# NVlabs/intrinsic3d

Measured on NVIDIA H100. Metric: gauss_newton_iterations_per_sec, higher is better.
Workload: dtype f32

## Files before the change

include/i3d_c_api.h:

```cpp
#ifndef I3D_C_API_H_
#define I3D_C_API_H_

#include <stdint.h>
#include "i3d_types.h"

#ifdef __cplusplus
extern "C" {
#endif

typedef struct I3DEngine I3DEngine;

int         i3d_abi_version(void);
uint64_t    i3d_sizeof_params(void);
uint64_t    i3d_sizeof_iter_info(void);

void        i3d_default_params(I3DParams* p);

int         i3d_engine_create(int device, I3DEngine** out);
void        i3d_engine_destroy(I3DEngine* e);
const char* i3d_last_error(const I3DEngine* e);

int         i3d_upload_grid(I3DEngine* e, int64_t n, const int32_t* xyz, const double* sdf0,
                            const double* sdf_refined, const double* albedo, const float* weight,
                            const uint8_t* rgb, float voxel_size);
// ... 47 lines not shown
int         i3d_mode_colors(I3DEngine* e, int32_t sdf_source, int32_t color_mode, uint8_t* rgb);
int         i3d_download_mesh(I3DEngine* e, float* xyz, uint8_t* rgb, int32_t* faces);

#define I3D_KEYFRAME_CHUNK 32
int         i3d_keyframe_scores(I3DEngine* e, int32_t F, int32_t W, int32_t H, const uint8_t* bgr, double* scores);
int         i3d_upload_rgbd_frames(I3DEngine* e, int32_t F, int32_t W, int32_t H, const uint8_t* bgr, const float* depth, const float* lum);
int         i3d_use_rgbd_level(I3DEngine* e, int32_t lvl, int32_t* W_out, int32_t* H_out);

int         i3d_sensor_frames_begin(I3DEngine* e, const I3DFusionCamera* depth_cam, const I3DFusionCamera* color_cam, int32_t capacity);
int         i3d_sensor_frames_add(I3DEngine* e, int32_t F, const float* depth, const uint8_t* bgr);
int32_t     i3d_sensor_num_frames(const I3DEngine* e);
int         i3d_sensor_keyframe_scores(I3DEngine* e, double* scores);
int         i3d_fusion_integrate_sensor(I3DEngine* e, int32_t n, const int32_t* ids, const float* pose_cam_to_world,
                                        const float* pose_world_to_cam);
int         i3d_select_rgbd_frames(I3DEngine* e, int32_t n, const int32_t* ids);

int         i3d_comm_unique_id(uint8_t id128[128]);
int         i3d_comm_init(I3DEngine* e, int32_t rank, int32_t world, const uint8_t id128[128]);
int         i3d_comm_p2p_export(I3DEngine* e, uint8_t handle64[64]);
int         i3d_comm_p2p_connect(I3DEngine* e, const uint8_t* handles );

int         i3d_set_shard(I3DEngine* e, int64_t voxel_begin, int64_t voxel_end);

double      i3d_phase_ms(const I3DEngine* e, const char* name);
int         i3d_debug_set_kernel_timers(I3DEngine* e, int level);
int64_t     i3d_phase_count(const I3DEngine* e, const char* name);
int64_t     i3d_debug_num_slots(const I3DEngine* e);
int         i3d_debug_set_keep_raw_jacobian(I3DEngine* e, int keep);
int         i3d_debug_get_rows(I3DEngine* e, int32_t* voxel, int32_t* frame, double* residual,
                               double* raw_weight, float* jac_colmajor);
int         i3d_debug_get_observations(I3DEngine* e, int32_t K, int32_t* frames, float* weights,
                                       uint8_t* active);
int         i3d_debug_get_step(I3DEngine* e, double* step, uint8_t* free_mask, double* col_scale);
int         i3d_debug_get_normal_equations(I3DEngine* e, float* b, float* s, float* jtj, float* cam_acc);
int         i3d_debug_apply_operator(I3DEngine* e, const float* v, float* q);
int64_t     i3d_debug_fusion_num_voxels(const I3DEngine* e);
int         i3d_debug_get_fusion_volume(I3DEngine* e, int32_t* xyz, float* sdf, float* weight, uint8_t* rgb);
int         i3d_debug_get_frames(I3DEngine* e, float* lum, float* depth, uint8_t* bgr);

#ifdef __cplusplus
}
#endif
#endif
```

intrinsic3d_b200/csrc/i3d_engine.cu:

```cuda
#include <cuda_runtime.h>
#include <dlfcn.h>

#include <algorithm>
#include <chrono>
#include <climits>
#include <cmath>
#include <cstdarg>
#include <cstdio>
#include <cstdlib>
#include <cstring>
#include <map>
#include <string>
#include <vector>

#include "../../include/i3d_c_api.h"
#include "i3d_kernels.cuh"
#include "i3d_lighting.cuh"
#include "i3d_recolor.cuh"
#include "i3d_gridops.cuh"
#include "i3d_fusion.cuh"
#include "i3d_frames.cuh"
#include "i3d_mesh.h"

#include <cub/device/device_radix_sort.cuh>
// ... 100 lines not shown
    Dev<float> Rt;
    Dev<FramePose> pose_ctx, pose_ctx_c;
    Dev<int32_t> obs_frame, row_frame;
    Dev<float> obs_w;
    Dev<float4> Jt;
    Dev<float2> Jtail;
    Dev<double> row_res, row_wraw;
    Dev<float> ea_w;
    Dev<double> lap;
    Dev<float> cam_acc;
    Dev<double> minv, type_w;
    Dev<int> fail_flag;
    Dev<float> v_bg, v_cg, v_s, v_jtj, v_b, v_x, v_r, v_z, v_p, v_ps, v_qg, v_tr, v_delta;
    Dev<double> v_bgd, v_cgd, v_qgd, cam_accd;
    Dev<CgCtl> ctl;
    Dev<double> red_partials, red_out;
    Dev<unsigned int> red_counters;
    size_t max_blocks = 0;
    bool keep_raw = false;
    Dev<float> dbg_v;
    I3DParams last_params{};
    bool have_iter = false;
    std::map<std::string, Phase> phases;
    cudaEvent_t ev[16];
    std::vector<cudaEvent_t> ev_pool;
    struct TimedLaunch { int a, b; const char* name; };
    std::vector<TimedLaunch> timed;
    size_t ev_used = 0;
    int64_t launches = 0;
    int64_t host_syncs = 0;
    int timer_level = 0;
    Dev<IterDev> iter_dev;
    int last_cg_iterations = 4, prev_cg_iterations = 4;
    Dev<uint8_t> color;
    bool have_color = false;
    Dev<unsigned long long> recolor_counts;
    Dev<int32_t> sv_table, sv_index, sv_nbr;
    Dev<int> sv_scalars, sv_deg;
    Dev<double> sv_acc, sv_work;
    Dev<I3DLightingInfo> sv_info;
    Dev<uint8_t> sh_has;
    int sv_S = 0;
    double* sv_x = nullptr;
    SubvolGrid sv_grid{};
    bool fu_active = false;
    I3DFusionParams fu_p{};
    uint64_t fu_cap = 0;
    int64_t fu_n = 0;
    Dev<unsigned long long> fu_keys; Dev<unsigned> fu_vals;
    Dev<int32_t> fu_x, fu_y, fu_z; Dev<float> fu_sdf, fu_w, fu_sdf2, fu_w2; Dev<uchar4> fu_rgb;
    Dev<int> fu_ctl;
    Dev<float> fu_depth_in, fu_depth, fu_nrm; Dev<uint8_t> fu_bgr;
    Dev<unsigned long long> fu_sk, fu_sk2; Dev<int32_t> fu_si, fu_si2; Dev<uint8_t> fu_cub;
    Dev<uint8_t> kf_bgr; Dev<double> kf_partials, kf_scores;
    int st_F = 0, st_W = 0, st_H = 0;
    Dev<float> st_lum, st_depth, st_tmp[4]; Dev<uint8_t> st_bgr;
    int sn_cap = 0, sn_F = 0;
    I3DFusionCamera sn_dcam{}, sn_ccam{};
    Dev<float> sn_depth; Dev<uint8_t> sn_bgr; Dev<int32_t> sn_ids;
    bool have_mesh = false;
    int64_t mesh_V = 0, mesh_F = 0;
    float* mesh_vpos = nullptr; uint8_t* mesh_vcol = nullptr; int3* mesh_faces = nullptr;
    Dev<uint8_t> ms_case, ms_keep, ms_cub; Dev<int32_t> ms_cnt, ms_sel; Dev<int64_t> ms_off; Dev<unsigned long long> ms_cubes, ms_best;
    Dev<float> ms_cpos, ms_vpos, ms_vpos2; Dev<uint8_t> ms_ccol, ms_vcol, ms_vcol2;
    Dev<uint32_t> ms_klo, ms_klo2; Dev<unsigned long long> ms_khi, ms_khi2;
    Dev<int32_t> ms_perm, ms_perm2, ms_first, ms_fid, ms_head, ms_seg, ms_cvid, ms_parent, ms_used, ms_newid;
// ... 419 lines not shown
    pdl_launch(e, k_pack, blocks_for(threads), kThreads, 0, shv, v0, v1, extra_f, n_extra_f, extra_d, n_extra_d, e->xbuf.p, e->ctl.p, respect_done);
    NK(g_nccl.AllReduce(e->xbuf.p, e->xbuf.p, total, NCCL_FLOAT64, NCCL_SUM, e->comm, e->stream));
    pdl_launch(e, k_unpack, blocks_for(threads), kThreads, 0, shv, v0, v1, extra_f, n_extra_f, extra_d, n_extra_d, e->xbuf.p, e->ctl.p, respect_done);
    e->launches += 2;
    if (epilogue_kind >= 0) { pdl_launch(e, k_epilogue, 1, 32, 0, e->ctl.p, extra_d, epilogue_kind, respect_done); e->launches += 1; }
}

size_t apply_smem_bytes(int F, int K)
{
    return static_cast<size_t>((6 * F + 9 + 15) & ~15) * sizeof(double) + static_cast<size_t>(14 + 6 * K) * kThreads * sizeof(float);
}

size_t accum_smem_bytes(int F, int K)
{
    return static_cast<size_t>((CamAccLayout{F}.size() + 15) & ~15) * sizeof(double) + static_cast<size_t>(K) * 8 * kThreads * sizeof(float);
}

int check_frame_limit(I3DEngine* e, int F, int K)
{
    int optin = 0;
    CK(cudaDeviceGetAttribute(&optin, cudaDevAttrMaxSharedMemoryPerBlockOptin, e->device));
    cudaFuncAttributes fa_acc{}, fa_app{};
    CK(cudaFuncGetAttributes(&fa_acc, k_eg_accum));
    CK(cudaFuncGetAttributes(&fa_app, k_eg_apply<APPLY_CG>));
    const size_t lim = static_cast<size_t>(optin);
    auto fits = [&](int f) { return fa_acc.sharedSizeBytes + accum_smem_bytes(f, K) <= lim && fa_app.sharedSizeBytes + apply_smem_bytes(f, K) <= lim; };
    if (fits(F)) return 0;
    int fmax = 0;
    while (fits(fmax + 1)) ++fmax;
    return fail(e, "i3d_gn_iteration: %d frames at K = %d observations need %zu bytes of shared memory per block in k_eg_accum (device limit %d): "
                   "at most %d frames at K = %d", F, K, fa_acc.sharedSizeBytes + accum_smem_bytes(F, K), optin, fmax, K);
}

void launch_operator(I3DEngine* e, const GridView& g, const RegView& rv, const EgRows& rows, const SolveVecs& sv, const Shard& sh, const float* vin,
                     float dmin, float dmax, int is_cg_iteration, bool sample_timing = false)
{
    if (rows.n_active > 0)
    {
        KernelTimer kt(e, "k_eg_apply", 0);
        pdl_launch(e, k_eg_apply<APPLY_CG>, blocks_for(rows.n_active), kThreads, apply_smem_bytes(e->F, rows.K), g, rows, rv, sv, sv.ps, e->ctl.p, 1, e->site(SITE_EG_APPLY));
    }
    e->launches += 2;
    {
        KernelTimer kt(e, "k_op_partial");
        pdl_launch(e, (k_op_partial<APPLY_CG, 4>), blocks_for(static_cast<size_t>((e->held_count() + 3) / 4)), kThreads, 0, 
            g, rv, sv, sh, e->held_count(), vin, sv.ps, e->type_w.p, dmin, dmax, e->ctl.p, 1, e->site(SITE_OP_POST), e->site(SITE_EG_APPLY).out, is_cg_iteration);
    }
    if (e->world > 1)
    {
        KernelTimer kt(e, "exchange");
        exchange(e, sv.qg, nullptr, sv.qg + 2 * e->n, 6 * e->F + 9, e->site(SITE_OP_POST).out, 1, 1, is_cg_iteration ? EPI_OPERATOR_CG : -1);
    }
}

int gn_iteration_impl(I3DEngine* e, const I3DParams& P, I3DIterInfo& info)
{
    std::memset(&info, 0, sizeof(info));
    if (e->n <= 0) return fail(e, "i3d_gn_iteration: no grid uploaded");
    if (e->F <= 0) return fail(e, "i3d_gn_iteration: no frames uploaded");
    if (!e->have_cam) return fail(e, "i3d_gn_iteration: camera not set");
    if (!e->have_sh) return fail(e, "i3d_gn_iteration: SH coefficients not set");
    if (e->world > 1 && !e->shard_ready) return fail(e, "i3d_gn_iteration: world > 1 but i3d_set_shard was not called after the grid/frames upload");
    int K = P.num_observations;
    if (K <= 0 || K > e->F) K = e->F;
    if (K > I3D_MAX_OBS) return fail(e, "i3d_gn_iteration: num_observations (%d) exceeds I3D_MAX_OBS (%d)", K, I3D_MAX_OBS);
    if (P.lm_steps < 1) return fail(e, "i3d_gn_iteration: lm_steps < 1");
    if (P.residual_reset_period < 1) return fail(e, "i3d_gn_iteration: residual_reset_period < 1");
    if (check_frame_limit(e, e->F, K) != 0) return 1;
    e->K = K;
    e->last_params = P;
    e->phases.clear(); e->timed.clear(); e->ev_used = 0; e->launches = 0; e->host_syncs = 0;
    const int64_t n = e->n;
    const int F = e->F;
    const bool multi = e->world > 1;
    cudaStream_t st = e->stream;
    ensure_vectors(e);
    e->iter_dev.ensure(1);
    const Shard sh = e->shard();
    const int64_t own = sh.own_end - sh.own_begin;
    const int64_t hc = e->held_count();
    const size_t U = static_cast<size_t>(e->U());
    Timer t_total(e, "total", 0);
    auto sync = [&]() { CK(cudaStreamSynchronize(st)); e->host_syncs += 1; };

    Timer t_sel(e, "select", 1);
// ... 98 lines not shown
    }
    if (multi) exchange(e, e->v_bg.p, e->v_cg.p, e->cam_acc.p, lay.size(), e->red_out.p, 2 * kSiteVals, 0);
    pdl_launch(e, k_type_weights, 1, 32, 0, e->iter_dev.p, e->site(SITE_BUILD).out, e->site(SITE_REG).out, P, n, e->type_w.p);
    if (S > 0) pdl_launch(e, k_row_weights, blocks_for(S), kThreads, 0, rows, e->type_w.p);
    SolveVecs sv = solve_vecs(e);
    pdl_launch(e, k_finish_problem, blocks_for(static_cast<size_t>((hc + 3) / 4)), kThreads, 0, g, rv, sv, sh, hc, e->type_w.p, e->cam_acc.p, P.fix_poses, P.fix_intrinsics,
                                                                              P.fix_distortion, P.gradient_tolerance, e->site(SITE_FINISH), e->cam);
    allreduce_scalars(e, e->site(SITE_FINISH).out, 3, -1, 0);
    pdl_launch(e, k_iter_finish, 1, 32, 0, e->iter_dev.p, e->site(SITE_FINISH).out, P);
    e->launches += 5;
    t_build.stop();
    e->have_iter = true;
    if (P.build_only)
    {
        IterDev hb{};
        CK(cudaMemcpyAsync(&hb, e->iter_dev.p, sizeof(hb), cudaMemcpyDeviceToHost, st));
        sync();
        CK(cudaGetLastError());
        info = hb.info;
        t_total.stop();
        return 0;
    }

    Timer t_solve(e, "solve", 3);
    const float dmin = static_cast<float>(P.min_lm_diagonal), dmax = static_cast<float>(std::min(P.max_lm_diagonal, 3.0e38));
    const unsigned upd_blocks = blocks_for(static_cast<size_t>((sh.held_voxel_unknowns() + 3) / 4 + F + 2));
    auto launch_update = [&](bool init, int refresh) {
        if (init) pdl_launch(e, (k_cg_update<true, 4>), upd_blocks, kThreads, 0, sv, sh, e->minv.p, dmin, dmax, e->ctl.p, refresh, e->site(SITE_UPDATE));
        else pdl_launch(e, (k_cg_update<false, 4>), upd_blocks, kThreads, 0, sv, sh, e->minv.p, dmin, dmax, e->ctl.p, refresh, e->site(SITE_UPDATE));
        e->launches += 1;
    };
    const unsigned vec_blocks = blocks_for(static_cast<size_t>(hc));
    const int max_it = P.forced_cg_iterations > 0 ? P.forced_cg_iterations : P.max_linear_solver_iterations;
    int enq = 0;
    auto enqueue_pcg = [&](int count) {
        for (int bidx = 0; bidx < count && enq < max_it; ++bidx)
        {
            ++enq;
            const bool refresh = (enq % P.residual_reset_period == 0);
            {
                KernelTimer kt(e, "k_cg_dir");
                pdl_launch(e, k_cg_dir4, blocks_for(static_cast<size_t>((hc + 3) / 4)), kThreads, 0, sv, sh, hc, e->ctl.p);
                e->launches += 1;
            }
            launch_operator(e, g, rv, rows, sv, sh, sv.p, dmin, dmax, 1, enq == 1);
            if (refresh)
            {
                pdl_launch(e, k_x_update, vec_blocks, kThreads, 0, sv, sh, hc, e->ctl.p);
                CK(cudaMemsetAsync(e->v_qg.p, 0, U * sizeof(float), st));
                pdl_launch(e, k_scale_vec, vec_blocks, kThreads, 0, sv, sh, hc, sv.x, 1.0f, sv.ps, e->ctl.p, 1);
                e->launches += 2;
                launch_operator(e, g, rv, rows, sv, sh, sv.x, dmin, dmax, 0);
                launch_update(false, 1);
            }
            else
            {
                KernelTimer kt(e, "k_cg_update");
                launch_update(false, 0);
            }
            if (multi) allreduce_scalars(e, e->site(SITE_UPDATE).out, 3, EPI_UPDATE, 1);
        }
    };
    auto enqueue_decision = [&]() {
        Timer t_cand(e, "candidate", 5);
        CK(cudaMemsetAsync(e->red_out.p + SITE_CAND * kSiteVals, 0, 3 * kSiteVals * sizeof(double), st));
        pdl_launch(e, k_candidate, vec_blocks, kThreads, 0, g, sv, sh, hc, 0, e->cam, e->c_sdf, e->c_alb, e->c_cam, e->v_delta.p, e->ctl.p, e->site(SITE_CAND));
        GridView gc = e->grid_view(e->c_sdf, e->c_alb);
        pdl_launch(e, k_frame_pose, blocks_for(F, 64), 64, 0, F, e->c_cam, e->pose_ctx_c.p);
        CamView cvc{e->c_cam, e->pose_ctx_c.p, F};
        if (n_active > 0)
        {
            KernelTimer kt(e, "k_eg_cost", 0);
            launch_eg_rows<ROWS_COST>(e, gc, cvc, rows, nullptr, nullptr);
        }
        pdl_launch(e, k_reg_cost, blocks_for(static_cast<size_t>(own)), kThreads, 0, gc, rv, sh, e->c_sdf, e->c_alb, e->site(SITE_REG_COST));
        if (multi) allreduce_scalars(e, e->red_out.p + SITE_CAND * kSiteVals, 3 * kSiteVals, -1, 0);
        pdl_launch(e, k_lm_decide, 1, 32, 0, e->iter_dev.p, e->ctl.p, e->fail_flag.p, e->site(SITE_CAND).out, e->site(SITE_EG_COST).out,
                                      e->site(SITE_REG_COST).out, e->type_w.p, P);
        e->launches += 5;
    };
    IterDev h{};
    for (int it = 1; it <= P.lm_steps; ++it)
    {
        Timer t_pcg(e, "pcg", 4);
        pdl_launch(e, k_lm_begin, 1, 32, 0, e->iter_dev.p, e->ctl.p, e->fail_flag.p, P);
        pdl_launch(e, k_cam_precond, blocks_for(static_cast<size_t>(F) + 2, 64), 64, 0, sv, e->cam_acc.p, e->type_w.p, e->ctl.p, dmin, dmax, e->minv.p, e->fail_flag.p);
        e->launches += 2;
        launch_update(true, 0);
        if (multi) allreduce_scalars(e, e->site(SITE_UPDATE).out, 3, EPI_UPDATE_INIT, 0);
        enq = 0;
        enqueue_pcg(P.forced_cg_iterations > 0 ? P.forced_cg_iterations : std::max(e->last_cg_iterations, e->prev_cg_iterations));
        t_pcg.stop();
        while (true)
        {
            enqueue_decision();
            CK(cudaMemcpyAsync(&h, e->iter_dev.p, sizeof(h), cudaMemcpyDeviceToHost, st));
            sync();
            CK(cudaGetLastError());
            if (!h.pcg_unfinished || h.state != LM_RUNNING) break;
            Timer t_more(e, "pcg", 4);
            enqueue_pcg(2);
        }
        if (h.info.lm_iterations >= 1)
        {
            e->prev_cg_iterations = e->last_cg_iterations;
            e->last_cg_iterations = std::max(1, h.info.cg_iterations[std::min(h.info.lm_iterations - 1, I3D_MAX_LM_STEPS - 1)]);
        }
        if (h.state != LM_RUNNING) break;
    }
    info = h.info;
    if (h.precond_fail) e->error = "camera preconditioner block not SPD";
    if (h.state == LM_ACCEPTED)
    {
        if (multi)
        {
            pdl_launch(e, k_mask_owned, blocks_for(U), kThreads, 0, sv, sh, e->v_delta.p);
            NK(g_nccl.AllReduce(e->v_delta.p, e->v_delta.p, U, NCCL_FLOAT32, NCCL_SUM, e->comm, st));
            pdl_launch(e, k_candidate, blocks_for(U), kThreads, 0, g, sv, sh, static_cast<int64_t>(U), 1, e->cam, e->c_sdf, e->c_alb, e->c_cam, e->v_delta.p, e->ctl.p,
                                                           e->site(SITE_CAND));
            sync();
            e->launches += 2;
// ... 227 lines not shown
}

extern "C" {

int i3d_abi_version(void) { return I3D_ABI_VERSION; }
uint64_t i3d_sizeof_params(void) { return sizeof(I3DParams); }
uint64_t i3d_sizeof_iter_info(void) { return sizeof(I3DIterInfo); }

void i3d_default_params(I3DParams* p)
{
    std::memset(p, 0, sizeof(*p));
    p->lambda[0] = 0.2; p->lambda[1] = 80.0; p->lambda[2] = 120.0; p->lambda[3] = 0.1;
    p->use_er = p->use_es = p->use_ea = 1;
    p->occlusion_distance = 0.02f; p->num_observations = 5; p->lm_steps = 50;
    p->initial_trust_region_radius = 1e4; p->max_trust_region_radius = 1e16; p->min_trust_region_radius = 1e-32;
    p->min_relative_decrease = 1e-3; p->min_lm_diagonal = 1e-6; p->max_lm_diagonal = 1e32; p->eta = 0.1;
    p->function_tolerance = 1e-6; p->gradient_tolerance = 1e-10; p->parameter_tolerance = 1e-8;
    p->max_linear_solver_iterations = 500; p->min_linear_solver_iterations = 0; p->residual_reset_period = 10;
    p->max_consecutive_invalid_steps = 5;
}

int i3d_engine_create(int device, I3DEngine** out)
{
    *out = nullptr;
    int count = 0;
    cudaError_t err = cudaGetDeviceCount(&count);
    if (err != cudaSuccess || count <= 0) return fail(nullptr, "i3d_engine_create: no CUDA device available (%s); this engine has no CPU fallback", cudaGetErrorString(err));
    if (device < 0 || device >= count) return fail(nullptr, "i3d_engine_create: device %d out of range (%d devices)", device, count);
    cudaDeviceProp prop;
    if (cudaGetDeviceProperties(&prop, device) != cudaSuccess) return fail(nullptr, "i3d_engine_create: cannot query device %d", device);
    if (prop.major != 9 || prop.minor != 0) return fail(nullptr, "i3d_engine_create: device %d is sm_%d%d; this library is built for sm_90a (H100) only", device, prop.major, prop.minor);
    I3DEngine* e = new I3DEngine();
    e->device = device;
    const int rc = guarded(e, [&]() {
        CK(cudaStreamCreateWithFlags(&e->stream, cudaStreamNonBlocking));
        for (auto& ev : e->ev) CK(cudaEventCreate(&ev));
        e->ev_pool.resize(4096);
        for (auto& ev : e->ev_pool) CK(cudaEventCreate(&ev));
        return 0;
    });
    if (rc != 0) { g_create_error = e->error; delete e; return rc; }
    *out = e;
    return 0;
}

void i3d_engine_destroy(I3DEngine* e)
{
    if (!e) return;
    cudaSetDevice(e->device);
    cudaStreamSynchronize(e->stream);
    for (size_t r = 0; r < e->peer_base.size(); ++r)
        if (static_cast<int>(r) != e->rank && e->peer_base[r]) cudaIpcCloseMemHandle(e->peer_base[r]);
    if (e->comm && g_nccl.CommDestroy) g_nccl.CommDestroy(e->comm);
    for (auto& ev : e->ev) cudaEventDestroy(ev);
    for (auto& ev : e->ev_pool) cudaEventDestroy(ev);
    if (e->ms_ev_ready) for (auto& ev : e->ms_ev) cudaEventDestroy(ev);
    cudaStreamDestroy(e->stream);
    delete e;
}

const char* i3d_last_error(const I3DEngine* e) { return e ? e->error.c_str() : g_create_error.c_str(); }

int i3d_upload_grid(I3DEngine* e, int64_t n, const int32_t* xyz, const double* sdf0, const double* sdf_refined, const double* albedo,
                    const float* weight, const uint8_t* rgb, float voxel_size)
{
    if (!e) return 1;
// ... 1079 lines not shown
        {
            std::vector<std::pair<std::pair<float, int>, int>> ord;
            for (int k = 0; k < K; ++k)
            {
                const size_t s = static_cast<size_t>(k) * e->stride + a;
                if (fr[s] >= 0) ord.push_back({{w[s], fr[s]}, k});
            }
            std::sort(ord.begin(), ord.end(), [](const auto& x, const auto& y) { return x.first > y.first; });
            for (size_t k = 0; k < ord.size(); ++k)
            {
                if (frames) frames[static_cast<size_t>(act[a]) * K + k] = ord[k].first.second;
                if (weights) weights[static_cast<size_t>(act[a]) * K + k] = ord[k].first.first;
            }
        }
        return 0;
    });
}

int i3d_debug_get_step(I3DEngine* e, double* step, uint8_t* free_mask, double* col_scale)
{
    if (!e || !e->have_iter) return fail(e, "i3d_debug_get_step: no iteration yet");
    return guarded(e, [&]() {
        const size_t U = static_cast<size_t>(e->U());
        std::vector<float> d(U), s(U);
        CK(cudaMemcpyAsync(d.data(), e->v_delta.p, U * sizeof(float), cudaMemcpyDeviceToHost, e->stream));
        CK(cudaMemcpyAsync(s.data(), e->v_s.p, U * sizeof(float), cudaMemcpyDeviceToHost, e->stream));
        CK(cudaStreamSynchronize(e->stream));
        for (size_t j = 0; j < U; ++j)
        {
            if (step) step[j] = d[j];
            if (free_mask) free_mask[j] = s[j] != 0.0f;
            if (col_scale) col_scale[j] = s[j];
        }
        return 0;
    });
}

int i3d_debug_get_normal_equations(I3DEngine* e, float* b, float* s, float* jtj, float* cam_acc)
{
    if (!e || !e->have_iter) return fail(e, "i3d_debug_get_normal_equations: no iteration yet");
    return guarded(e, [&]() {
        const size_t U = static_cast<size_t>(e->U());
        cudaStream_t st = e->stream;
        if (b) CK(cudaMemcpyAsync(b, e->v_b.p, U * sizeof(float), cudaMemcpyDeviceToHost, st));
        if (s) CK(cudaMemcpyAsync(s, e->v_s.p, U * sizeof(float), cudaMemcpyDeviceToHost, st));
        if (jtj) CK(cudaMemcpyAsync(jtj, e->v_jtj.p, U * sizeof(float), cudaMemcpyDeviceToHost, st));
        if (cam_acc) CK(cudaMemcpyAsync(cam_acc, e->cam_acc.p, CamAccLayout{e->F}.size() * sizeof(float), cudaMemcpyDeviceToHost, st));
        CK(cudaStreamSynchronize(st));
        return 0;
    });
}

int i3d_debug_apply_operator(I3DEngine* e, const float* v, float* q)
{
    if (!e || !e->have_iter) return fail(e, "i3d_debug_apply_operator: no iteration yet");
    if (!v || !q) return fail(e, "i3d_debug_apply_operator: NULL vector");
    if (e->world > 1) return fail(e, "i3d_debug_apply_operator: single GPU only");
    return guarded(e, [&]() {
        cudaStream_t st = e->stream;
        const size_t U = static_cast<size_t>(e->U());
        const I3DParams& P = e->last_params;
        e->dbg_v.ensure(U);
        CgCtl saved{}, running{};
        CK(cudaMemcpyAsync(&saved, e->ctl.p, sizeof(CgCtl), cudaMemcpyDeviceToHost, st));
        CK(cudaStreamSynchronize(st));
        running = saved; running.done = 0; running.inv_radius = 0.0;
// ... 56 lines not shown
```

intrinsic3d_b200/csrc/i3d_kernels.cuh:

```cuda
#pragma once
#include <cuda_runtime.h>
#include <stdint.h>
#include <limits.h>
#include "i3d_math.cuh"
#include "i3d_grid.cuh"
#include "../../include/i3d_types.h"

namespace i3d
{

enum : uint8_t { FL_VALID = 1, FL_ACTIVE = 2, FL_RING = 4, FL_FREE_SDF = 8, FL_FREE_ALB = 16, FL_ES_JAC = 32, FL_ROW = 64  };

struct Shard
{
    int64_t own_begin, own_end;
    int64_t hv0, hv1;
    int cam_owner;
    int defer;
    int64_t loc_begin, loc_end;
    __device__ __forceinline__ bool owns_voxel(int64_t v) const { return v >= own_begin && v < own_end; }
    __device__ __forceinline__ bool owns_unknown(int64_t j, int64_t n) const
    {
        return j < n ? owns_voxel(j) : (j < 2 * n ? owns_voxel(j - n) : cam_owner != 0);
    }
    __host__ __device__ __forceinline__ int64_t held_voxel_unknowns() const { return 2 * (hv1 - hv0); }
    __device__ __forceinline__ int64_t unknown(int64_t t, int64_t n) const
    {
        const int64_t L = hv1 - hv0;
        return t < L ? hv0 + t : (t < 2 * L ? n + hv0 + (t - L) : 2 * n + (t - 2 * L));
    }
    __device__ __forceinline__ bool vec4(int64_t e0, int64_t n, int64_t* j0) const
    {
        const int64_t L = hv1 - hv0;
        if (e0 + 4 > 2 * L) return false;
// ... 1759 lines not shown
            a0 += static_cast<double>(rr[i]) * ssum;
        }
        if (sh.cam_owner) { acc[0] = a0; acc[1] = a1; acc[2] = a2; }
    }
    if (grid_reduce<3>(acc, site) && threadIdx.x == 0 && !sh.defer) epilogue_update(ctl, site.out[0], site.out[1], site.out[2], INIT);
}

__global__ void __launch_bounds__(kThreads)
k_cg_dir4(SolveVecs sv, Shard sh, int64_t count, const CgCtl* __restrict__ ctl)
{
    pdl_prologue();
    if (ctl->done) return;
    const int64_t e0 = (blockIdx.x * static_cast<int64_t>(blockDim.x) + threadIdx.x) * 4;
    if (e0 >= count) return;
    const float beta = static_cast<float>(ctl->beta);
    int64_t j0 = 0;
    if (sh.vec4(e0, sv.n, &j0))
    {
        float z[4], p[4], s4[4], ps[4];
        ld4(sv.z, j0, z); ld4(sv.p, j0, p); ld4(sv.s, j0, s4);
#pragma unroll
        for (int i = 0; i < 4; ++i) { p[i] = (beta == 0.0f) ? z[i] : z[i] + beta * p[i]; ps[i] = s4[i] * p[i]; }
        st4(sv.p, j0, p); st4(sv.ps, j0, ps);
    }
    else
        for (int64_t t = e0; t < e0 + 4 && t < count; ++t)
        {
            const int64_t j = sh.unknown(t, sv.n);
            const float p = (beta == 0.0f) ? sv.z[j] : sv.z[j] + beta * sv.p[j];
            sv.p[j] = p; sv.ps[j] = sv.s[j] * p;
        }
}

struct ShareView
{
    int64_t n_shared;
    const int32_t* slist;
    const uint8_t* held;
};

__global__ void k_pack(ShareView sh, const float* __restrict__ v0, const float* __restrict__ v1, const float* __restrict__ extra_f, int n_extra_f,
                       const double* __restrict__ extra_d, int n_extra_d, double* __restrict__ xbuf, const CgCtl* __restrict__ ctl, int respect_done)
{
    pdl_prologue();
    if (respect_done && ctl->done) return;
    const int64_t t = blockIdx.x * static_cast<int64_t>(blockDim.x) + threadIdx.x;
    const int64_t nv = v1 ? 2 : 1;
    if (t < sh.n_shared)
    {
        const int32_t j = sh.slist[t];
        const bool h = sh.held[j] != 0;
        xbuf[t] = h ? static_cast<double>(v0[j]) : 0.0;
        if (v1) xbuf[sh.n_shared + t] = h ? static_cast<double>(v1[j]) : 0.0;
    }
    else if (t < sh.n_shared + n_extra_f) xbuf[nv * sh.n_shared + (t - sh.n_shared)] = static_cast<double>(extra_f[t - sh.n_shared]);
    else if (t < sh.n_shared + n_extra_f + n_extra_d) xbuf[nv * sh.n_shared + (t - sh.n_shared)] = extra_d[t - sh.n_shared - n_extra_f];
}

__global__ void k_unpack(ShareView sh, float* __restrict__ v0, float* __restrict__ v1, float* __restrict__ extra_f, int n_extra_f,
                         double* __restrict__ extra_d, int n_extra_d, const double* __restrict__ xbuf, const CgCtl* __restrict__ ctl, int respect_done)
{
    pdl_prologue();
    if (respect_done && ctl->done) return;
    const int64_t t = blockIdx.x * static_cast<int64_t>(blockDim.x) + threadIdx.x;
    const int64_t nv = v1 ? 2 : 1;
    if (t < sh.n_shared)
// ... 348 lines not shown
```

intrinsic3d_b200/engine.py:

```python
from __future__ import annotations

import ctypes as C
import os

import numpy as np

from .ctypes_defs import (I3DFusionCamera, I3DFusionParams, I3DIterInfo, I3DLightingInfo, I3DLightingParams, I3DMeshInfo, I3DMeshParams,
                          I3DParams)

_HERE = os.path.dirname(os.path.abspath(__file__))
LIB_PATH = os.environ.get("I3D_LIB", os.path.join(_HERE, "libi3d_b200.so"))
_LIB = None

EXPORTED_SYMBOLS = [
    "i3d_abi_version", "i3d_sizeof_params", "i3d_sizeof_iter_info", "i3d_default_params",
    "i3d_engine_create", "i3d_engine_destroy", "i3d_last_error",
    "i3d_upload_grid", "i3d_upload_voxel_params", "i3d_upload_frames", "i3d_set_camera", "i3d_set_sh",
    "i3d_gn_iteration", "i3d_download_state",
    "i3d_sizeof_lighting_params", "i3d_sizeof_lighting_info", "i3d_default_lighting_params", "i3d_estimate_lighting",
    "i3d_lighting_num_subvolumes", "i3d_download_lighting", "i3d_download_voxel_sh",
    "i3d_upload_color_frames", "i3d_recompute_colors", "i3d_download_colors",
    "i3d_num_voxels", "i3d_clear_voxels_outside_thin_shell", "i3d_upsample_grid", "i3d_download_grid",
    "i3d_sizeof_fusion_params", "i3d_default_fusion_params", "i3d_fusion_begin", "i3d_fusion_integrate", "i3d_fusion_finish",
    "i3d_keyframe_scores", "i3d_upload_rgbd_frames", "i3d_use_rgbd_level",
    "i3d_sensor_frames_begin", "i3d_sensor_frames_add", "i3d_sensor_num_frames", "i3d_sensor_keyframe_scores", "i3d_fusion_integrate_sensor",
    "i3d_select_rgbd_frames",
    "i3d_sizeof_mesh_info", "i3d_extract_mesh", "i3d_download_mesh", "i3d_extract_mesh_colored", "i3d_mode_colors",
    "i3d_comm_unique_id", "i3d_comm_init", "i3d_comm_p2p_export", "i3d_comm_p2p_connect", "i3d_set_shard",
    "i3d_phase_ms", "i3d_phase_count", "i3d_debug_set_kernel_timers", "i3d_debug_num_slots", "i3d_debug_set_keep_raw_jacobian",
    "i3d_debug_get_rows", "i3d_debug_get_observations", "i3d_debug_get_step", "i3d_debug_get_normal_equations",
    "i3d_debug_apply_operator", "i3d_debug_fusion_num_voxels", "i3d_debug_get_fusion_volume", "i3d_debug_get_frames",
]
KEYFRAME_CHUNK = 32
COLOR_MODES = {"": 0, "normals": 1, "lap": 2, "lum": 3, "lum_grad": 4, "albedo": 5, "shading_sv": 6, "shading_sv_const": 7, "chroma": 8}


def load_library():
    global _LIB
    if _LIB is not None:
        return _LIB
    if not os.path.exists(LIB_PATH):
        raise RuntimeError(f"{LIB_PATH} not found: build it with intrinsic3d_b200/csrc/build.sh "
                           "(__graft_entry__.build()); there is no CPU fallback")
    L = C.CDLL(LIB_PATH)
    L.i3d_abi_version.restype = C.c_int
    L.i3d_sizeof_params.restype = C.c_uint64
    L.i3d_sizeof_iter_info.restype = C.c_uint64
    L.i3d_last_error.restype = C.c_char_p
    L.i3d_last_error.argtypes = [C.c_void_p]
    L.i3d_phase_ms.restype = C.c_double
    L.i3d_phase_ms.argtypes = [C.c_void_p, C.c_char_p]
    L.i3d_phase_count.restype = C.c_int64
    L.i3d_phase_count.argtypes = [C.c_void_p, C.c_char_p]
    L.i3d_debug_num_slots.restype = C.c_int64
    L.i3d_debug_num_slots.argtypes = [C.c_void_p]
    L.i3d_sizeof_lighting_params.restype = C.c_uint64
    L.i3d_sizeof_lighting_info.restype = C.c_uint64
    L.i3d_lighting_num_subvolumes.restype = C.c_int64
    L.i3d_lighting_num_subvolumes.argtypes = [C.c_void_p]
    L.i3d_num_voxels.restype = C.c_int64
    L.i3d_num_voxels.argtypes = [C.c_void_p]
    L.i3d_sizeof_fusion_params.restype = C.c_uint64
    L.i3d_debug_fusion_num_voxels.restype = C.c_int64
# ... 326 lines not shown

    def phase_count(self, name: str) -> int:
        return int(self.L.i3d_phase_count(self.h, name.encode()))

    def set_kernel_timers(self, level: int):
        self.L.i3d_debug_set_kernel_timers(self.h, C.c_int(int(level)))

    def debug_rows(self, want_jac=True):
        S = int(self.L.i3d_debug_num_slots(self.h))
        voxel = np.empty(S, np.int32)
        frame = np.empty(S, np.int32)
        res = np.empty(S, np.float64)
        w = np.empty(S, np.float64)
        J = np.empty((29, S), np.float32) if want_jac else None
        self._check(self.L.i3d_debug_get_rows(self.h, _p(voxel, C.c_int32), _p(frame, C.c_int32), _p(res, C.c_double), _p(w, C.c_double),
                                              _p(J, C.c_float)))
        return dict(voxel=voxel, frame=frame, residual=res, raw_weight=w, J=J)

    def debug_observations(self, K: int):
        fr = np.empty((self.n, K), np.int32)
        w = np.empty((self.n, K), np.float32)
        act = np.empty(self.n, np.uint8)
        self._check(self.L.i3d_debug_get_observations(self.h, C.c_int32(K), _p(fr, C.c_int32), _p(w, C.c_float), _p(act, C.c_uint8)))
        return fr, w, act

    def debug_step(self):
        U = 2 * self.n + 6 * self.F + 9
        st = np.zeros(U, np.float64)
        fm = np.zeros(U, np.uint8)
        cs = np.zeros(U, np.float64)
        self._check(self.L.i3d_debug_get_step(self.h, _p(st, C.c_double), _p(fm, C.c_uint8), _p(cs, C.c_double)))
        return st, fm, cs

    def debug_normal_equations(self):
        U = 2 * self.n + 6 * self.F + 9
        b, s, jtj = np.empty(U, np.float32), np.empty(U, np.float32), np.empty(U, np.float32)
        cam = np.empty(33 * self.F + 43, np.float32)
        self._check(self.L.i3d_debug_get_normal_equations(self.h, _p(b, C.c_float), _p(s, C.c_float), _p(jtj, C.c_float), _p(cam, C.c_float)))
        return dict(b=b, s=s, jtj=jtj, cam_acc=cam)

    def debug_apply_operator(self, v):
        U = 2 * self.n + 6 * self.F + 9
        v = np.ascontiguousarray(v, np.float32)
        assert v.shape == (U,)
        q = np.empty(U, np.float32)
        self._check(self.L.i3d_debug_apply_operator(self.h, _p(v, C.c_float), _p(q, C.c_float)))
        return q


def shard_range(n: int, rank: int, world: int, align: int = 512):
    if world <= 1:
        return 0, n
    per = -(-n // world)
    per = -(-per // align) * align
    b = min(n, rank * per)
    e = min(n, (rank + 1) * per)
    if rank == world - 1:
        e = n
    return b, e


def cut_ranges(cost, world: int, align: int = 64):
    import torch
    n = int(cost.shape[0])
    c = torch.cumsum(cost.to(torch.float64), 0)
    total = float(c[-1].item()) if n > 0 else 0.0
# ... 105 lines not shown
```

Before: 133.9.

## Fuse PCG operator epilogue, update and direction into one cooperative kernel

```diff
diff --git a/include/i3d_c_api.h b/include/i3d_c_api.h
--- a/include/i3d_c_api.h
+++ b/include/i3d_c_api.h
@@ -103,6 +103,7 @@
 int         i3d_debug_get_observations(I3DEngine* e, int32_t K, int32_t* frames, float* weights,
                                        uint8_t* active);
 int         i3d_debug_get_step(I3DEngine* e, double* step, uint8_t* free_mask, double* col_scale);
+int         i3d_debug_get_pcg_vectors(I3DEngine* e, float* x, float* p);
 int         i3d_debug_get_normal_equations(I3DEngine* e, float* b, float* s, float* jtj, float* cam_acc);
 int         i3d_debug_apply_operator(I3DEngine* e, const float* v, float* q);
 int64_t     i3d_debug_fusion_num_voxels(const I3DEngine* e);
diff --git a/intrinsic3d_b200/csrc/i3d_engine.cu b/intrinsic3d_b200/csrc/i3d_engine.cu
--- a/intrinsic3d_b200/csrc/i3d_engine.cu
+++ b/intrinsic3d_b200/csrc/i3d_engine.cu
@@ -156,6 +156,9 @@
     int timer_level = 0;
     Dev<IterDev> iter_dev;
     int last_cg_iterations = 4, prev_cg_iterations = 4;
+    bool pcg_fused = true;
+    int64_t step_n = -1;
+    unsigned step_grid = 0; int step_K = 0; size_t step_smem = 0;
     Dev<uint8_t> color;
     bool have_color = false;
     Dev<unsigned long long> recolor_counts;
@@ -641,15 +644,21 @@
                    "at most %d frames at K = %d", F, K, fa_acc.sharedSizeBytes + accum_smem_bytes(F, K), optin, fmax, K);
 }
 
+void launch_eg_apply(I3DEngine* e, const GridView& g, const RegView& rv, const EgRows& rows, const SolveVecs& sv)
+{
+    if (rows.n_active > 0)
+    {
+        KernelTimer kt(e, "k_eg_apply", 0);
+        pdl_launch(e, k_eg_apply<APPLY_CG>, blocks_for(rows.n_active), kThreads, apply_smem_bytes(e->F, rows.K), g, rows, rv, sv, sv.ps, e->ctl.p, 1, e->site(SITE_EG_APPLY));
+    }
+    e->launches += 1;
+}
+
 void launch_operator(I3DEngine* e, const GridView& g, const RegView& rv, const EgRows& rows, const SolveVecs& sv, const Shard& sh, const float* vin,
                      float dmin, float dmax, int is_cg_iteration, bool sample_timing = false)
 {
-    if (rows.n_active > 0)
-    {
-        KernelTimer kt(e, "k_eg_apply", 0);
-        pdl_launch(e, k_eg_apply<APPLY_CG>, blocks_for(rows.n_active), kThreads, apply_smem_bytes(e->F, rows.K), g, rows, rv, sv, sv.ps, e->ctl.p, 1, e->site(SITE_EG_APPLY));
-    }
-    e->launches += 2;
+    launch_eg_apply(e, g, rv, rows, sv);
+    e->launches += 1;
     {
         KernelTimer kt(e, "k_op_partial");
         pdl_launch(e, (k_op_partial<APPLY_CG, 4>), blocks_for(static_cast<size_t>((e->held_count() + 3) / 4)), kThreads, 0, 
@@ -660,6 +669,55 @@
         KernelTimer kt(e, "exchange");
         exchange(e, sv.qg, nullptr, sv.qg + 2 * e->n, 6 * e->F + 9, e->site(SITE_OP_POST).out, 1, 1, is_cg_iteration ? EPI_OPERATOR_CG : -1);
     }
+}
+
+bool plan_cg_step(I3DEngine* e)
+{
+    if (e->step_n == e->n) return e->step_grid > 0;
+    e->step_n = e->n; e->step_grid = 0;
+    int sms = 0, optin = 0;
+    CK(cudaDeviceGetAttribute(&sms, cudaDevAttrMultiProcessorCount, e->device));
+    CK(cudaDeviceGetAttribute(&optin, cudaDevAttrMaxSharedMemoryPerBlockOptin, e->device));
+    cudaFuncAttributes fa0{}, fa1{};
+    CK(cudaFuncGetAttributes(&fa0, k_cg_step<false>));
+    CK(cudaFuncGetAttributes(&fa1, k_cg_step<true>));
+    const size_t dyn_max = static_cast<size_t>(optin) - std::max(fa0.sharedSizeBytes, fa1.sharedSizeBytes);
+    CK(cudaFuncSetAttribute(k_cg_step<false>, cudaFuncAttributeMaxDynamicSharedMemorySize, static_cast<int>(dyn_max)));
+    CK(cudaFuncSetAttribute(k_cg_step<true>, cudaFuncAttributeMaxDynamicSharedMemorySize, static_cast<int>(dyn_max)));
+    const int64_t items = (e->n + 3) / 4;
+    for (int bps = 2048 / kStepThreads; bps >= 1; --bps)
+    {
+        const int64_t threads = static_cast<int64_t>(bps) * sms * kStepThreads;
+        const int64_t K = (items + threads - 1) / threads;
+        const size_t smem = static_cast<size_t>(K) * kStepSlots * kStepThreads * sizeof(float);
+        if (smem > dyn_max) break;
+        int occ0 = 0, occ1 = 0;
+        CK(cudaOccupancyMaxActiveBlocksPerMultiprocessor(&occ0, k_cg_step<false>, kStepThreads, smem));
+        CK(cudaOccupancyMaxActiveBlocksPerMultiprocessor(&occ1, k_cg_step<true>, kStepThreads, smem));
+        if (std::min(occ0, occ1) < bps) continue;
+        if (static_cast<size_t>(bps) * sms + 8 > e->max_blocks) break;
+        e->step_grid = static_cast<unsigned>(bps * sms); e->step_K = static_cast<int>(K); e->step_smem = smem;
+        return true;
+    }
+    return false;
+}
+
+template <bool INIT>
+void launch_cg_step(I3DEngine* e, const GridView& g, const RegView& rv, const SolveVecs& sv, float dmin, float dmax)
+{
+    static const bool pdl = [] { const char* v = std::getenv("I3D_PDL"); return !(v && v[0] == '0'); }();
+    cudaLaunchConfig_t cfg{};
+    cfg.gridDim = dim3(e->step_grid); cfg.blockDim = dim3(kStepThreads); cfg.dynamicSmemBytes = e->step_smem; cfg.stream = e->stream;
+    cudaLaunchAttribute at[2];
+    at[0].id = cudaLaunchAttributeCooperative;
+    at[0].val.cooperative = 1;
+    at[1].id = cudaLaunchAttributeProgrammaticStreamSerialization;
+    at[1].val.programmaticStreamSerializationAllowed = 1;
+    cfg.attrs = at; cfg.numAttrs = pdl ? 2 : 1;
+    const int64_t items = (e->n + 3) / 4;
+    CK(cudaLaunchKernelEx(&cfg, k_cg_step<INIT>, g, rv, sv, items, e->step_K, static_cast<const double*>(e->type_w.p), static_cast<const double*>(e->minv.p),
+                          dmin, dmax, e->ctl.p, e->site(SITE_OP_POST), static_cast<const double*>(e->site(SITE_EG_APPLY).out), e->site(SITE_UPDATE)));
+    e->launches += 1;
 }
 
 int gn_iteration_impl(I3DEngine* e, const I3DParams& P, I3DIterInfo& info)
@@ -824,16 +882,28 @@
     };
     const unsigned vec_blocks = blocks_for(static_cast<size_t>(hc));
     const int max_it = P.forced_cg_iterations > 0 ? P.forced_cg_iterations : P.max_linear_solver_iterations;
+    const bool fused = e->pcg_fused && !multi && plan_cg_step(e);
     int enq = 0;
+    bool dir_ready = false;
     auto enqueue_pcg = [&](int count) {
         for (int bidx = 0; bidx < count && enq < max_it; ++bidx)
         {
             ++enq;
             const bool refresh = (enq % P.residual_reset_period == 0);
+            if (!dir_ready)
             {
                 KernelTimer kt(e, "k_cg_dir");
                 pdl_launch(e, k_cg_dir4, blocks_for(static_cast<size_t>((hc + 3) / 4)), kThreads, 0, sv, sh, hc, e->ctl.p);
                 e->launches += 1;
+            }
+            dir_ready = false;
+            if (fused && !refresh)
+            {
+                launch_eg_apply(e, g, rv, rows, sv);
+                KernelTimer kt(e, "k_cg_update");
+                launch_cg_step<false>(e, g, rv, sv, dmin, dmax);
+                dir_ready = true;
+                continue;
             }
             launch_operator(e, g, rv, rows, sv, sh, sv.p, dmin, dmax, 1, enq == 1);
             if (refresh)
@@ -878,7 +948,9 @@
         pdl_launch(e, k_lm_begin, 1, 32, 0, e->iter_dev.p, e->ctl.p, e->fail_flag.p, P);
         pdl_launch(e, k_cam_precond, blocks_for(static_cast<size_t>(F) + 2, 64), 64, 0, sv, e->cam_acc.p, e->type_w.p, e->ctl.p, dmin, dmax, e->minv.p, e->fail_flag.p);
         e->launches += 2;
-        launch_update(true, 0);
+        if (fused) launch_cg_step<true>(e, g, rv, sv, dmin, dmax);
+        else launch_update(true, 0);
+        dir_ready = fused;
         if (multi) allreduce_scalars(e, e->site(SITE_UPDATE).out, 3, EPI_UPDATE_INIT, 0);
         enq = 0;
         enqueue_pcg(P.forced_cg_iterations > 0 ? P.forced_cg_iterations : std::max(e->last_cg_iterations, e->prev_cg_iterations));
@@ -1172,6 +1244,7 @@
     if (prop.major != 9 || prop.minor != 0) return fail(nullptr, "i3d_engine_create: device %d is sm_%d%d; this library is built for sm_90a (H100) only", device, prop.major, prop.minor);
     I3DEngine* e = new I3DEngine();
     e->device = device;
+    { const char* v = std::getenv("I3D_PCG_FUSED"); e->pcg_fused = !(v && v[0] == '0'); }
     const int rc = guarded(e, [&]() {
         CK(cudaStreamCreateWithFlags(&e->stream, cudaStreamNonBlocking));
         for (auto& ev : e->ev) CK(cudaEventCreate(&ev));
@@ -2317,6 +2390,18 @@
             if (free_mask) free_mask[j] = s[j] != 0.0f;
             if (col_scale) col_scale[j] = s[j];
         }
+        return 0;
+    });
+}
+
+int i3d_debug_get_pcg_vectors(I3DEngine* e, float* x, float* p)
+{
+    if (!e || !e->have_iter) return fail(e, "i3d_debug_get_pcg_vectors: no iteration yet");
+    return guarded(e, [&]() {
+        const size_t U = static_cast<size_t>(e->U());
+        if (x) CK(cudaMemcpyAsync(x, e->v_x.p, U * sizeof(float), cudaMemcpyDeviceToHost, e->stream));
+        if (p) CK(cudaMemcpyAsync(p, e->v_p.p, U * sizeof(float), cudaMemcpyDeviceToHost, e->stream));
+        CK(cudaStreamSynchronize(e->stream));
         return 0;
     });
 }
diff --git a/intrinsic3d_b200/csrc/i3d_kernels.cuh b/intrinsic3d_b200/csrc/i3d_kernels.cuh
--- a/intrinsic3d_b200/csrc/i3d_kernels.cuh
+++ b/intrinsic3d_b200/csrc/i3d_kernels.cuh
@@ -1,5 +1,6 @@
 #pragma once
 #include <cuda_runtime.h>
+#include <cooperative_groups.h>
 #include <stdint.h>
 #include <limits.h>
 #include "i3d_math.cuh"
@@ -1825,6 +1826,328 @@
         }
 }
 
+constexpr int kStepThreads = 256;
+constexpr int kStepSlots = 8;
+
+__device__ __forceinline__ void ld4n(const float* __restrict__ p, int64_t j, int cnt, bool vec, float (&v)[4])
+{
+    if (vec) { ld4(p, j, v); return; }
+#pragma unroll
+    for (int i = 0; i < 4; ++i) v[i] = i < cnt ? p[j + i] : 0.0f;
+}
+__device__ __forceinline__ void st4n(float* __restrict__ p, int64_t j, int cnt, bool vec, const float (&v)[4])
+{
+    if (vec) { st4(p, j, v); return; }
+#pragma unroll
+    for (int i = 0; i < 4; ++i) if (i < cnt) p[j + i] = v[i];
+}
+
+template <int NV>
+__device__ __forceinline__ void step_partials(const double (&vals)[NV], double* __restrict__ partials, double* red_smem)
+{
+#pragma unroll
+    for (int i = 0; i < NV; ++i)
+    {
+        const double s = block_sum<double>(vals[i], red_smem);
+        if (threadIdx.x == 0) partials[static_cast<size_t>(blockIdx.x) * NV + i] = s;
+    }
+}
+template <int NV>
+__device__ __forceinline__ void step_totals(const double* __restrict__ partials, double (&tot)[NV])
+{
+#pragma unroll
+    for (int i = 0; i < NV; ++i)
+    {
+        double s = 0.0;
+        for (unsigned int b = threadIdx.x; b < gridDim.x; b += 32) s += __ldcg(&partials[static_cast<size_t>(b) * NV + i]);
+        tot[i] = warp_sum(s);
+    }
+}
+
+template <bool INIT>
+__global__ void __launch_bounds__(kStepThreads, 3)
+k_cg_step(GridView g, RegView rv, SolveVecs sv, int64_t items, int K, const double* __restrict__ type_w, const double* __restrict__ minv,
+          float dmin, float dmax, CgCtl* __restrict__ ctl, ReduceSite op_site, const double* __restrict__ eg_partial, ReduceSite upd_site)
+{
+    extern __shared__ float s_slot[];
+    __shared__ CgCtl s_ctl;
+    __shared__ double red_smem[32];
+    pdl_prologue();
+    cooperative_groups::grid_group grid = cooperative_groups::this_grid();
+    const int tid = threadIdx.x;
+    if (tid == 0) s_ctl = *ctl;
+    __syncthreads();
+    if (!INIT && s_ctl.done) return;
+    const int64_t n = sv.n;
+    const int64_t T = static_cast<int64_t>(gridDim.x) * blockDim.x;
+    const int64_t gt = blockIdx.x * static_cast<int64_t>(blockDim.x) + tid;
+    const float inv_radius = static_cast<float>(s_ctl.inv_radius);
+    const int64_t tail0 = (2 * n) & ~int64_t(3);
+    auto slot = [&](int k, int u) -> float& { return s_slot[(k * kStepSlots + u) * blockDim.x + tid]; };
+
+    const int64_t cblk = T - 1 - gt;
+    int m = 0; int64_t cbase = 0; const double* Mi = nullptr;
+    if (cblk < sv.F + 2)
+    {
+        const int blk = static_cast<int>(cblk);
+        const int64_t n2 = 2 * n;
+        if (blk < sv.F) { m = 6; cbase = n2 + 6 * static_cast<int64_t>(blk); Mi = minv + 36 * static_cast<size_t>(blk); }
+        else if (blk == sv.F) { m = 4; cbase = n2 + 6 * static_cast<int64_t>(sv.F); Mi = minv + 36 * static_cast<size_t>(sv.F); }
+        else { m = 5; cbase = n2 + 6 * static_cast<int64_t>(sv.F) + 4; Mi = minv + 36 * static_cast<size_t>(sv.F) + 16; }
+    }
+
+    if (!INIT)
+    {
+        double acc[1] = {0.0};
+        const float wr = static_cast<float>(type_w[1]), ws = static_cast<float>(type_w[2]), wa = static_cast<float>(type_w[3]);
+        const float* __restrict__ ps = sv.ps;
+        for (int k = 0; k < K; ++k)
+        {
+            const int64_t item = gt + k * T;
+            if (item >= items) break;
+            const int64_t v0 = 4 * item;
+            const int cnt = n - v0 < 4 ? static_cast<int>(n - v0) : 4;
+            float regs[2][4];
+#pragma unroll
+            for (int i = 0; i < 4; ++i)
+            {
+                regs[0][i] = 0.0f; regs[1][i] = 0.0f;
+                if (i >= cnt) continue;
+                const int64_t v = v0 + i;
+                int32_t nb[6];
+#pragma unroll
+                for (int o = 0; o < 6; ++o) nb[o] = (rv.use_er || rv.use_ea) ? g.nbr[static_cast<int64_t>(o) * n + v] : -1;
+                float reg = 0.0f;
+                if (rv.use_er)
+                {
+                    const float t0 = sv.tr[v];
+                    float tt;
+                    if (i < 2 && nb[0] >= 0) tt = __fmaf_rn(t0, -6.0f, sv.tr[nb[0]]);
+                    else { tt = __fmul_rn(t0, -6.0f); if (nb[0] >= 0) tt = __fadd_rn(tt, sv.tr[nb[0]]); }
+#pragma unroll
+                    for (int o = 1; o < 6; ++o) if (nb[o] >= 0) tt = __fadd_rn(tt, sv.tr[nb[o]]);
+                    reg = __fmaf_rn(wr, tt, reg);
+                    acc[0] += static_cast<double>(wr) * t0 * t0;
+                }
+                const uint8_t fl = rv.flags[v];
+                if (rv.use_es && (fl & FL_ACTIVE) && (fl & FL_ES_JAC))
+                {
+                    const float u = ps[v];
+                    reg = __fmaf_rn(ws, u, reg);
+                    acc[0] += static_cast<double>(ws) * u * u;
+                }
+                regs[0][i] = reg;
+                reg = 0.0f;
+                if (rv.use_ea)
+                {
+                    const float pa = ps[n + v];
+#pragma unroll
+                    for (int d = 0; d < 3; ++d)
+                    {
+                        const float wp = rv.ea_w[static_cast<int64_t>(d) * n + v];
+                        if (wp != 0.0f)
+                        {
+                            const float du = __fsub_rn(pa, ps[n + nb[2 * d]]);
+                            reg = __fmaf_rn(__fmul_rn(wa, wp), du, reg);
+                            acc[0] += static_cast<double>(wa) * wp * du * du;
+                        }
+                        const int32_t mm = nb[2 * d + 1];
+                        if (mm >= 0)
+                        {
+                            const float wm = rv.ea_w[static_cast<int64_t>(d) * n + mm];
+                            if (wm != 0.0f) reg = __fmaf_rn(__fmul_rn(wa, wm), __fsub_rn(pa, ps[n + mm]), reg);
+                        }
+                    }
+                }
+                regs[1][i] = reg;
+            }
+#pragma unroll
+            for (int h = 0; h < 2; ++h)
+            {
+                const int64_t j0 = h * n + v0;
+                const bool vec = cnt == 4 && (h == 0 || (n & 3) == 0);
+                float pj[4], jt[4], sj[4];
+                double eg[4];
+                ld4n(sv.p, j0, cnt, vec, pj); ld4n(sv.jtj, j0, cnt, vec, jt); ld4n(sv.s, j0, cnt, vec, sj);
+                if (vec)
+                {
+                    const double2 e01 = *reinterpret_cast<const double2*>(sv.qgd + j0), e23 = *reinterpret_cast<const double2*>(sv.qgd + j0 + 2);
+                    eg[0] = e01.x; eg[1] = e01.y; eg[2] = e23.x; eg[3] = e23.y;
+                }
+                else
+                {
+#pragma unroll
+                    for (int i = 0; i < 4; ++i) eg[i] = i < cnt ? sv.qgd[j0 + i] : 0.0;
+                }
+#pragma unroll
+                for (int i = 0; i < 4; ++i)
+                {
+                    if (i >= cnt) continue;
+                    if (eg[i] != 0.0) sv.qgd[j0 + i] = 0.0;
+                    const float add = __fadd_rn(static_cast<float>(eg[i]), regs[h][i]);
+                    const float qg = (add != 0.0f) ? add : 0.0f;
+                    const float d2 = __fmul_rn(lm_diag(jt[i], dmin, dmax), inv_radius);
+                    acc[0] += static_cast<double>(d2) * pj[i] * pj[i];
+                    slot(k, 4 * h + i) = (j0 + i < tail0) ? __fmaf_rn(sj[i], qg, __fmul_rn(d2, pj[i])) : __fmaf_rn(d2, pj[i], __fmul_rn(sj[i], qg));
+                }
+            }
+        }
+#pragma unroll
+        for (int k = 0; k < 6; ++k)
+        {
+            if (k >= m) break;
+            const int64_t j = cbase + k;
+            const double eg = sv.qgd[j];
+            if (eg != 0.0) sv.qgd[j] = 0.0;
+            const float add = __fadd_rn(static_cast<float>(eg), 0.0f);
+            const float qg = (add != 0.0f) ? add : 0.0f;
+            const float pj = sv.p[j];
+            const float d2 = __fmul_rn(lm_diag(sv.jtj[j], dmin, dmax), inv_radius);
+            acc[0] += static_cast<double>(d2) * pj * pj;
+            sv.z[j] = __fmaf_rn(d2, pj, __fmul_rn(sv.s[j], qg));
+        }
+        step_partials<1>(acc, op_site.partials, red_smem);
+        grid.sync();
+        if (tid < 32)
+        {
+            double tot[1];
+            step_totals<1>(op_site.partials, tot);
+            if (tid == 0)
+            {
+                const double total = tot[0] + eg_partial[0];
+                epilogue_operator(&s_ctl, total, APPLY_CG, 1);
+                if (blockIdx.x == 0) { op_site.out[0] = total; if (s_ctl.done) *ctl = s_ctl; }
+            }
+        }
+        __syncthreads();
+        if (s_ctl.done) return;
+    }
+
+    {
+        double acc[3] = {0.0, 0.0, 0.0};
+        const float alpha = INIT ? 0.0f : static_cast<float>(s_ctl.alpha);
+        for (int k = 0; k < K; ++k)
+        {
+            const int64_t item = gt + k * T;
+            if (item >= items) break;
+            const int64_t v0 = 4 * item;
+            const int cnt = n - v0 < 4 ? static_cast<int>(n - v0) : 4;
+#pragma unroll
+            for (int h = 0; h < 2; ++h)
+            {
+                const int64_t j0 = h * n + v0;
+                const bool vec = cnt == 4 && (h == 0 || (n & 3) == 0);
+                float bj[4], jt[4], vj[4], xo[4], ro[4], xn[4], rn[4];
+                ld4n(sv.b, j0, cnt, vec, bj); ld4n(sv.jtj, j0, cnt, vec, jt);
+                if (!INIT) { ld4n(sv.p, j0, cnt, vec, vj); ld4n(sv.x, j0, cnt, vec, xo); ld4n(sv.r, j0, cnt, vec, ro); }
+#pragma unroll
+                for (int i = 0; i < 4; ++i)
+                {
+                    const float d2 = __fmul_rn(lm_diag(jt[i], dmin, dmax), inv_radius);
+                    if (INIT) { xn[i] = 0.0f; rn[i] = bj[i]; }
+                    else
+                    {
+                        const float qj = (i < cnt) ? slot(k, 4 * h + i) : 0.0f;
+                        xn[i] = __fmaf_rn(alpha, vj[i], xo[i]);
+                        rn[i] = __fmaf_rn(-alpha, qj, ro[i]);
+                    }
+                    if (i >= cnt) continue;
+                    const float zn = __fdiv_rn(rn[i], __fadd_rn(jt[i], d2));
+                    slot(k, 4 * h + i) = zn;
+                    acc[0] += static_cast<double>(rn[i]) * zn;
+                    acc[1] -= static_cast<double>(xn[i]) * (static_cast<double>(bj[i]) + rn[i]);
+                    acc[2] += static_cast<double>(d2) * xn[i] * xn[i];
+                }
+                st4n(sv.x, j0, cnt, vec, xn); st4n(sv.r, j0, cnt, vec, rn);
+            }
+        }
+        if (m > 0)
+        {
+            float rr[6];
+            double a0 = 0.0, a1 = 0.0, a2 = 0.0;
+#pragma unroll
+            for (int k = 0; k < 6; ++k)
+            {
+                rr[k] = 0.0f;
+                if (k >= m) continue;
+                const int64_t j = cbase + k;
+                const float bj = sv.b[j];
+                const float d2 = __fmul_rn(lm_diag(sv.jtj[j], dmin, dmax), inv_radius);
+                float xj, rj;
+                if (INIT) { xj = 0.0f; rj = bj; }
+                else
+                {
+                    const float vj = sv.p[j];
+                    xj = __fmaf_rn(alpha, vj, sv.x[j]);
+                    rj = __fmaf_rn(-alpha, sv.z[j], sv.r[j]);
+                }
+                sv.x[j] = xj; sv.r[j] = rj; rr[k] = rj;
+                a1 -= static_cast<double>(xj) * (static_cast<double>(bj) + rj);
+                a2 += static_cast<double>(d2) * xj * xj;
+            }
+#pragma unroll
+            for (int i = 0; i < 6; ++i)
+            {
+                if (i >= m) continue;
+                double ssum = 0.0;
+#pragma unroll
+                for (int k = 0; k < 6; ++k) if (k < m) ssum += Mi[i * m + k] * static_cast<double>(rr[k]);
+                sv.z[cbase + i] = static_cast<float>(ssum);
+                a0 += static_cast<double>(rr[i]) * ssum;
+            }
+            acc[0] += a0; acc[1] += a1; acc[2] += a2;
+        }
+        step_partials<3>(acc, upd_site.partials, red_smem);
+        grid.sync();
+        if (tid < 32)
+        {
+            double tot[3];
+            step_totals<3>(upd_site.partials, tot);
+            if (tid == 0)
+            {
+                epilogue_update(&s_ctl, tot[0], tot[1], tot[2], INIT);
+                if (blockIdx.x == 0) { upd_site.out[0] = tot[0]; upd_site.out[1] = tot[1]; upd_site.out[2] = tot[2]; *ctl = s_ctl; }
+            }
+        }
+        __syncthreads();
+        if (s_ctl.done) return;
+    }
+
+    const float beta = static_cast<float>(s_ctl.beta);
+    for (int k = 0; k < K; ++k)
+    {
+        const int64_t item = gt + k * T;
+        if (item >= items) break;
+        const int64_t v0 = 4 * item;
+        const int cnt = n - v0 < 4 ? static_cast<int>(n - v0) : 4;
+#pragma unroll
+        for (int h = 0; h < 2; ++h)
+        {
+            const int64_t j0 = h * n + v0;
+            const bool vec = cnt == 4 && (h == 0 || (n & 3) == 0);
+            float p[4], s4[4], ps[4];
+            ld4n(sv.s, j0, cnt, vec, s4);
+            if (beta != 0.0f) ld4n(sv.p, j0, cnt, vec, p);
+#pragma unroll
+            for (int i = 0; i < 4; ++i)
+            {
+                const float z = (i < cnt) ? slot(k, 4 * h + i) : 0.0f;
+                p[i] = (beta == 0.0f) ? z : __fmaf_rn(beta, p[i], z);
+                ps[i] = __fmul_rn(s4[i], p[i]);
+            }
+            st4n(sv.p, j0, cnt, vec, p); st4n(sv.ps, j0, cnt, vec, ps);
+        }
+    }
+#pragma unroll
+    for (int k = 0; k < 6; ++k)
+    {
+        if (k >= m) break;
+        const int64_t j = cbase + k;
+        const float p = (beta == 0.0f) ? sv.z[j] : __fmaf_rn(beta, sv.p[j], sv.z[j]);
+        sv.p[j] = p; sv.ps[j] = __fmul_rn(sv.s[j], p);
+    }
+}
+
 struct ShareView
 {
     int64_t n_shared;
diff --git a/intrinsic3d_b200/engine.py b/intrinsic3d_b200/engine.py
--- a/intrinsic3d_b200/engine.py
+++ b/intrinsic3d_b200/engine.py
@@ -28,7 +28,7 @@
     "i3d_sizeof_mesh_info", "i3d_extract_mesh", "i3d_download_mesh", "i3d_extract_mesh_colored", "i3d_mode_colors",
     "i3d_comm_unique_id", "i3d_comm_init", "i3d_comm_p2p_export", "i3d_comm_p2p_connect", "i3d_set_shard",
     "i3d_phase_ms", "i3d_phase_count", "i3d_debug_set_kernel_timers", "i3d_debug_num_slots", "i3d_debug_set_keep_raw_jacobian",
-    "i3d_debug_get_rows", "i3d_debug_get_observations", "i3d_debug_get_step", "i3d_debug_get_normal_equations",
+    "i3d_debug_get_rows", "i3d_debug_get_observations", "i3d_debug_get_step", "i3d_debug_get_pcg_vectors", "i3d_debug_get_normal_equations",
     "i3d_debug_apply_operator", "i3d_debug_fusion_num_voxels", "i3d_debug_get_fusion_volume", "i3d_debug_get_frames",
 ]
 KEYFRAME_CHUNK = 32
@@ -421,6 +421,12 @@
         self._check(self.L.i3d_debug_get_step(self.h, _p(st, C.c_double), _p(fm, C.c_uint8), _p(cs, C.c_double)))
         return st, fm, cs
 
+    def debug_pcg_vectors(self):
+        U = 2 * self.n + 6 * self.F + 9
+        x, p = np.empty(U, np.float32), np.empty(U, np.float32)
+        self._check(self.L.i3d_debug_get_pcg_vectors(self.h, _p(x, C.c_float), _p(p, C.c_float)))
+        return x, p
+
     def debug_normal_equations(self):
         U = 2 * self.n + 6 * self.F + 9
         b, s, jtj = np.empty(U, np.float32), np.empty(U, np.float32), np.empty(U, np.float32)
```

Result: faster. 138.4, median of 6 (+3.4%).
